# shionhonda/IaGo

Hardware: AMD Instinct MI355X
Metric: self-play games/sec (higher is better)
Workload: dtype f16 MFMA operands (float32 split in 2 / 3 pieces), f32 accumulate; u64 bitboards; f32 / f64 tree statistics

## Files before the change

iago_amd/csrc/conv_policy_body.hpp:

```cpp
#pragma once
#include "abi_common.hpp"
#include "search_request.hpp"

#include <hip/hip_fp16.h>

#include <cstdlib>

#include <atomic>

namespace iago_policy {


typedef _Float16 half8 __attribute__((ext_vector_type(8)));
typedef float float16v __attribute__((ext_vector_type(16)));
typedef float float4v __attribute__((ext_vector_type(4)));
#define IAGO_POLICY_MFMA16(acc, a, b) asm volatile("v_mfma_f32_16x16x32_f16 %0, %1, %2, %0" : "+a"(acc) : "v"(a), "v"(b))
typedef unsigned int u32x4 __attribute__((ext_vector_type(4)));
typedef float f2 __attribute__((ext_vector_type(2)));
typedef _Float16 h2 __attribute__((ext_vector_type(2)));

constexpr int RS = 800;
constexpr int ZB = 1280;
constexpr int BS = 64 * RS + ZB;
constexpr int HEAD_FLOATS = 64;
constexpr int W1_LDS = (64 * 18 + 64) * 4;
constexpr int LDS_BYTES = BS + 1024 + HEAD_FLOATS * 4 + W1_LDS;
constexpr float S1 = 1.0f / 2048.0f, S2 = 1.0f / (2048.0f * 2048.0f);

struct PolicyParams {
    const uint64_t *own, *opp;
    const int64_t *index;
    const int32_t *n_dev;
    int64_t n;
    const float *w1, *b1;
    const uint4 *w_hi[7], *w_mid[7], *w_lo[7];
    const float *bias[7];
    const float *w9, *b10;
    float *probs;
    uint32_t *overflow;
    int layer_lo, layer_hi;
    uint4 *scratch;
    int64_t row_lo, row_hi;
};

__device__ __forceinline__ void split3(const f2 v, h2 &hi, h2 &mid, h2 &lo)
{
    hi = __builtin_convertvector(v, h2);
    const f2 r1 = (v - __builtin_convertvector(hi, f2)) * 2048.0f;
    mid = __builtin_convertvector(r1, h2);
    const f2 r2 = (r1 - __builtin_convertvector(mid, f2)) * 2048.0f;
    lo = __builtin_convertvector(r2, h2);
}

extern __shared__ __align__(16) char policy_lds[];

template <bool SRCH = false>
__device__ __forceinline__ void policy_item(const PolicyParams &P, const int64_t row_id, const uint32_t *pos = nullptr,
                                            float *res = nullptr, const float *w1_staged = nullptr,
                                            const float *head_w = nullptr)
{
    char *const T = policy_lds;
    int tid_ = threadIdx.x;
    if constexpr (SRCH)
        asm volatile("" : "+v"(tid_));
    const int tid = tid_, wv = __builtin_amdgcn_readfirstlane(tid >> 6), lane = tid & 63;
    const int64_t b = P.index ? P.index[row_id] : row_id;

    if (tid < ZB / 16)
        *(uint4 *)(T + 64 * RS + tid * 16) = make_uint4(0, 0, 0, 0);
    bool saturated = false;
    if (P.layer_lo > 0) {
        const uint4 *src = P.scratch + (row_id - P.row_lo) * (64 * RS / 16);
        for (int e = tid; e < 64 * RS / 16; e += 256)
            *(uint4 *)(T + e * 16) = src[e];
    } else {
        const int cell = tid & 63, y = cell >> 3, x = cell & 7;
        const uint64_t bits0 = SRCH ? iago_request::opp(pos) : P.opp[b];
        const uint64_t bits1 = SRCH ? iago_request::own(pos) : P.own[b];
        float in[18];
#pragma unroll
        for (int c = 0; c < 2; c++)
#pragma unroll
            for (int ky = 0; ky < 3; ky++)
#pragma unroll
                for (int kx = 0; kx < 3; kx++) {
                    const int yy = y + ky - 1, xx = x + kx - 1;
                    const bool ok = yy >= 0 && yy < 8 && xx >= 0 && xx < 8;
                    const int a = (yy * 8 + xx) & 63;
                    in[c * 9 + ky * 3 + kx] = (ok && (((c ? bits1 : bits0) >> a) & 1ull)) ? 1.0f : 0.0f;
                }
        const float *w1s = w1_staged;
        if constexpr (!SRCH) {
            float *const st = (float *)(T + BS + 1024 + HEAD_FLOATS * 4);
            for (int e = tid; e < 64 * 18 / 4; e += 256)
                ((float4 *)st)[e] = ((const float4 *)P.w1)[e];
            if (tid < 16)
                ((float4 *)(st + 64 * 18))[tid] = ((const float4 *)P.b1)[tid];
            __syncthreads();
            w1s = st;
        }
#pragma unroll 1
        for (int g2 = 0; g2 < 2; g2++) {
            const int grp = __builtin_amdgcn_readfirstlane(g2 * 4 + wv);
            const int co0 = grp * 8;
            _Float16 p0[8], p1[8], p2[8];
#pragma unroll
            for (int k = 0; k < 8; k += 2) {
                const float *wa = w1s + (co0 + k) * 18, *wb = wa + 18;
                f2 acc = (f2){w1s[64 * 18 + co0 + k], w1s[64 * 18 + co0 + k + 1]};
#pragma unroll
                for (int j = 0; j < 18; j++)
                    acc = __builtin_elementwise_fma((f2){wa[j], wb[j]}, (f2){in[j], in[j]}, acc);
                saturated |= !(acc.x <= 65000.0f) || !(acc.y <= 65000.0f);
                f2 v;
                v.x = fminf(fmaxf(acc.x, 0.0f), 65000.0f);
                v.y = fminf(fmaxf(acc.y, 0.0f), 65000.0f);
                h2 a0, a1, a2;
                split3(v, a0, a1, a2);
                p0[k] = a0.x, p0[k + 1] = a0.y;
                p1[k] = a1.x, p1[k + 1] = a1.y;
                p2[k] = a2.x, p2[k + 1] = a2.y;
            }
            char *dst = T + cell * RS + (grp >> 1) * 32 + (grp & 1) * 16;
            *(uint4 *)dst = *(const uint4 *)p0;
            *(uint4 *)(dst + 256) = *(const uint4 *)p1;
            *(uint4 *)(dst + 512) = *(const uint4 *)p2;
        }
    }
    __syncthreads();

    const int c16 = lane & 15, kq = lane >> 4;
    uint32_t addr[4][9];
#pragma unroll
    for (int q = 0; q < 4; q++)
#pragma unroll
        for (int tap = 0; tap < 9; tap++) {
            const int cell = 16 * q + c16;
            const int yy = (cell >> 3) + tap / 3 - 1, xx = (cell & 7) + tap % 3 - 1;
            const bool ok = yy >= 0 && yy < 8 && xx >= 0 && xx < 8;
            const int lin = (cell + (tap / 3 - 1) * 8 + (tap % 3 - 1)) & 7;
            addr[q][tap] = (uint32_t)((ok ? (yy * 8 + xx) * RS : 64 * RS + 32 * lin) + kq * 16);
        }
    uint32_t wrow[4];
#pragma unroll
    for (int q = 0; q < 4; q++)
        wrow[q] = (uint32_t)((16 * q + c16) * RS);

    for (int L = P.layer_lo; L < P.layer_hi; L++) {
        const int n_pairs = L == 0 ? 2 : 4;
        const char *const wh = (const char *)P.w_hi[L], *const wm = (const char *)P.w_mid[L], *const wl = (const char *)P.w_lo[L];
        const uint32_t a_lane = (uint32_t)(((32 * wv + c16) * 2 + (kq & 1) + (kq >> 1) * (9 * 256)) * 16);
        auto a_load = [&](const char *base, uint32_t step_bytes, int m) -> u32x4 {
            return *(const u32x4 *)(base + step_bytes + a_lane + (uint32_t)m * 512u);
        };
        float4v acc0[2][4], acc0b[2][4], acc1[2][4], acc2[2][4];
#pragma unroll
        for (int m = 0; m < 2; m++)
#pragma unroll
            for (int n = 0; n < 4; n++)
#pragma unroll
                for (int v = 0; v < 4; v++) {
                    acc0[m][n][v] = 0.0f;
                    acc0b[m][n][v] = 0.0f;
                    acc1[m][n][v] = 0.0f;
                    acc2[m][n][v] = 0.0f;
                }
        u32x4 a_hi[3][2], a_mid[3][2], a_lo[3][2];
#pragma unroll
        for (int i = 0; i < 2; i++)
#pragma unroll
            for (int m = 0; m < 2; m++) {
                a_hi[i][m] = a_load(wh, (uint32_t)i * 4096u, m);
                a_mid[i][m] = a_load(wm, (uint32_t)i * 4096u, m);
                a_lo[i][m] = a_load(wl, (uint32_t)i * 4096u, m);
            }
        half8 bh[3], bm[3], bl[3];
        auto b_addr = [&](int tile) -> const char * {
            const int over = tile >= 36 ? 64 : 0, tt = tile % 36;
            return T + addr[tt & 3][tt >> 2] + over;
        };
        {
            const char *p0 = b_addr(0), *p1 = b_addr(1);
            bh[0] = *(const half8 *)p0, bm[0] = *(const half8 *)(p0 + 256), bl[0] = *(const half8 *)(p0 + 512);
            bh[1] = *(const half8 *)p1, bm[1] = *(const half8 *)(p1 + 256), bl[1] = *(const half8 *)(p1 + 512);
        }
        for (int cp = 0; cp < n_pairs; cp++) {
#pragma unroll
            for (int tap = 0; tap < 9; tap++) {
                int cp2 = cp, tp2 = tap + 2;
                if (tp2 >= 9) {
                    tp2 -= 9;
                    cp2 += 1;
                }
                if (cp2 >= n_pairs) {
                    cp2 = n_pairs - 1;
                    tp2 = 8;
                }
                const uint32_t w2 = (uint32_t)(18 * cp2 + tp2) * 4096u;
                half8 ah[2], am[2], al[2];
#pragma unroll
                for (int m = 0; m < 2; m++) {
                    ah[m] = __builtin_bit_cast(half8, a_hi[tap % 3][m]);
                    am[m] = __builtin_bit_cast(half8, a_mid[tap % 3][m]);
                    al[m] = __builtin_bit_cast(half8, a_lo[tap % 3][m]);
                }
#pragma unroll
                for (int q = 0; q < 4; q++) {
                    const int tile = tap * 4 + q, cur = tile % 3, nxt = (tile + 2) % 3;
                    const char *p = b_addr(tile + 2);
                    __builtin_amdgcn_sched_barrier(0);
                    IAGO_POLICY_MFMA16(acc2[0][q], ah[0], bl[cur]);
                    bh[nxt] = *(const half8 *)p;
                    __builtin_amdgcn_sched_barrier(0);
                    IAGO_POLICY_MFMA16(acc2[1][q], ah[1], bl[cur]);
                    bm[nxt] = *(const half8 *)(p + 256);
                    __builtin_amdgcn_sched_barrier(0);
                    IAGO_POLICY_MFMA16(acc1[0][q], ah[0], bm[cur]);
                    bl[nxt] = *(const half8 *)(p + 512);
                    __builtin_amdgcn_sched_barrier(0);
                    IAGO_POLICY_MFMA16(acc1[1][q], ah[1], bm[cur]);
                    if (q == 0)
                        a_hi[(tap + 2) % 3][0] = a_load(wh, w2, 0);
                    else if (q == 1)
                        a_mid[(tap + 2) % 3][0] = a_load(wm, w2, 0);
                    else if (q == 2)
                        a_lo[(tap + 2) % 3][0] = a_load(wl, w2, 0);
                    __builtin_amdgcn_sched_barrier(0);
                    if (tap & 1)
                        IAGO_POLICY_MFMA16(acc0b[0][q], ah[0], bh[cur]);
                    else
                        IAGO_POLICY_MFMA16(acc0[0][q], ah[0], bh[cur]);
                    if (q == 0)
                        a_hi[(tap + 2) % 3][1] = a_load(wh, w2, 1);
                    else if (q == 1)
                        a_mid[(tap + 2) % 3][1] = a_load(wm, w2, 1);
                    else if (q == 2)
                        a_lo[(tap + 2) % 3][1] = a_load(wl, w2, 1);
                    __builtin_amdgcn_sched_barrier(0);
                    if (tap & 1)
                        IAGO_POLICY_MFMA16(acc0b[1][q], ah[1], bh[cur]);
                    else
                        IAGO_POLICY_MFMA16(acc0[1][q], ah[1], bh[cur]);
                    IAGO_POLICY_MFMA16(acc2[0][q], al[0], bh[cur]);
                    IAGO_POLICY_MFMA16(acc2[1][q], al[1], bh[cur]);
                    IAGO_POLICY_MFMA16(acc1[0][q], am[0], bh[cur]);
                    IAGO_POLICY_MFMA16(acc1[1][q], am[1], bh[cur]);
                    IAGO_POLICY_MFMA16(acc2[0][q], am[0], bm[cur]);
                    IAGO_POLICY_MFMA16(acc2[1][q], am[1], bm[cur]);
                    __builtin_amdgcn_sched_barrier(0);
                }
            }
#pragma unroll
            for (int q = 0; q < 4; q++)
#pragma unroll
                for (int tap = 0; tap < 9; tap++)
                    addr[q][tap] += 64u;
        }
#pragma unroll
        for (int q = 0; q < 4; q++)
#pragma unroll
            for (int tap = 0; tap < 9; tap++)
                addr[q][tap] -= 64u * (uint32_t)n_pairs;

        f2 bia[2][2];
#pragma unroll
        for (int m = 0; m < 2; m++) {
            const float4 bq = *(const float4 *)(P.bias[L] + 32 * wv + 16 * m + 4 * kq);
            bia[m][0] = (f2){bq.x, bq.y};
            bia[m][1] = (f2){bq.z, bq.w};
        }
        asm volatile("s_nop 15\n\ts_nop 7" ::: "memory");
        __syncthreads();
        float vmax = 0.0f;
        f2 vsum = (f2){0.0f, 0.0f};
#pragma unroll
        for (int q = 0; q < 4; q++) {
            char *row = T + wrow[q] + (32 * wv + 4 * kq) * 2;
#pragma unroll
            for (int m = 0; m < 2; m++) {
                h2 p0[2], p1[2], p2[2];
#pragma unroll
                for (int t2 = 0; t2 < 2; t2++) {
                    const f2 m0 = (f2){acc0[m][q][2 * t2], acc0[m][q][2 * t2 + 1]} + (f2){acc0b[m][q][2 * t2], acc0b[m][q][2 * t2 + 1]};
                    const f2 m1 = (f2){acc1[m][q][2 * t2], acc1[m][q][2 * t2 + 1]};
                    const f2 m2 = (f2){acc2[m][q][2 * t2], acc2[m][q][2 * t2 + 1]};
                    f2 v = (m2 * S2 + m1 * S1) + m0 + bia[m][t2];
                    vmax = fmaxf(fmaxf(vmax, v.x), v.y);
                    vsum += v;
                    v.x = __builtin_amdgcn_fmed3f(v.x, 0.0f, 65000.0f);
                    v.y = __builtin_amdgcn_fmed3f(v.y, 0.0f, 65000.0f);
                    split3(v, p0[t2], p1[t2], p2[t2]);
                }
                *(uint2 *)(row + 32 * m) = (uint2){__builtin_bit_cast(uint32_t, p0[0]), __builtin_bit_cast(uint32_t, p0[1])};
                *(uint2 *)(row + 32 * m + 256) =
                    (uint2){__builtin_bit_cast(uint32_t, p1[0]), __builtin_bit_cast(uint32_t, p1[1])};
                *(uint2 *)(row + 32 * m + 512) =
                    (uint2){__builtin_bit_cast(uint32_t, p2[0]), __builtin_bit_cast(uint32_t, p2[1])};
            }
        }
        saturated |= !(vmax <= 65000.0f) || !(vsum.x + vsum.y == vsum.x + vsum.y);
        __syncthreads();
    }
    if (P.overflow && saturated)
        *P.overflow = 1u;
    if (P.layer_hi < 7) {
        uint4 *dst = P.scratch + (row_id - P.row_lo) * (64 * RS / 16);
        for (int e = tid; e < 64 * RS / 16; e += 256)
            dst[e] = *(const uint4 *)(T + e * 16);
        return;
    }

    if (wv == 0) {
        const char *row = T + lane * RS;
        float acc = 0.0f;
#pragma unroll 4
        for (int c8 = 0; c8 < 16; c8++) {
            const half8 xh = *(const half8 *)(row + c8 * 16), xm = *(const half8 *)(row + 256 + c8 * 16),
                        xl = *(const half8 *)(row + 512 + c8 * 16);
            const float *w9 = SRCH ? head_w : P.w9;
            const float4 wa = *(const float4 *)(w9 + c8 * 8), wb = *(const float4 *)(w9 + c8 * 8 + 4);
            const float w[8] = {wa.x, wa.y, wa.z, wa.w, wb.x, wb.y, wb.z, wb.w};
#pragma unroll
            for (int e = 0; e < 8; e++) {
                const float xv = ((float)xl[e] * S2 + (float)xm[e] * S1) + (float)xh[e];
                acc = fmaf(w[e], xv, acc);
            }
        }
        const float logit = acc + (SRCH ? head_w[128 + lane] : P.b10[lane]);
        float mx = logit;
#pragma unroll
        for (int o = 32; o > 0; o >>= 1)
            mx = fmaxf(mx, __shfl_xor(mx, o));
        const float e = expf(logit - mx);
        float sum = e;
#pragma unroll
        for (int o = 32; o > 0; o >>= 1)
            sum += __shfl_xor(sum, o);
        if constexpr (SRCH)
            res[lane] = e / sum;
        else
            P.probs[row_id * 64 + lane] = e / sum;
    }
}

inline int policy_params_of(const iago_policy_split3_args *a, PolicyParams &P)
{
    if (!a || a->n < 0)
        return iago_fail(IAGO_ERR_INVALID, "iago_policy_forward_split3: null args or n < 0");
    if (!a->own || !a->opp || !a->w1 || !a->b1 || !a->w9 || !a->b10 || !a->probs)
        return iago_fail(IAGO_ERR_INVALID, "iago_policy_forward_split3: null pointer");
    for (int L = 0; L < 7; L++) {
        if (!a->w_hi[L] || !a->w_mid[L] || !a->w_lo[L] || !a->bias[L] || ((uintptr_t)a->w_hi[L] & 15u) ||
            ((uintptr_t)a->w_mid[L] & 15u) || ((uintptr_t)a->w_lo[L] & 15u) || ((uintptr_t)a->bias[L] & 15u))
            return iago_fail(IAGO_ERR_INVALID, "iago_policy_forward_split3: weights and biases of blocks 2..8 must be "
                                               "non-null and 16-byte aligned");
        P.w_hi[L] = (const uint4 *)a->w_hi[L];
        P.w_mid[L] = (const uint4 *)a->w_mid[L];
        P.w_lo[L] = (const uint4 *)a->w_lo[L];
        P.bias[L] = a->bias[L];
    }
    if (((uintptr_t)a->w9 & 15u) || ((uintptr_t)a->w1 & 15u) || ((uintptr_t)a->b1 & 15u))
        return iago_fail(IAGO_ERR_INVALID, "iago_policy_forward_split3: w1, b1, w9 must be 16-byte aligned");
    P.own = a->own;
    P.opp = a->opp;
    P.index = a->index;
    P.n_dev = a->n_dev;
    P.n = a->n;
    P.w1 = a->w1;
    P.b1 = a->b1;
    P.w9 = a->w9;
    P.b10 = a->b10;
    P.probs = a->probs;
    P.overflow = a->overflow;
    P.layer_lo = 0;
    P.layer_hi = 7;
    P.scratch = nullptr;
    P.row_lo = 0;
    P.row_hi = a->n;
    return IAGO_OK;
}

}
```

iago_amd/csrc/conv_trunk_body.hpp:

```cpp
#pragma once
#include "abi_common.hpp"
#include "rollout_row_body.hpp"
#include "search_request.hpp"

#include <hip/hip_fp16.h>

#include <atomic>
#include <type_traits>

namespace iago_trunk {


typedef _Float16 half8 __attribute__((ext_vector_type(8)));
typedef float float16v __attribute__((ext_vector_type(16)));
typedef float float4v __attribute__((ext_vector_type(4)));
typedef unsigned int u32x4 __attribute__((ext_vector_type(4)));
typedef float f2 __attribute__((ext_vector_type(2)));
typedef _Float16 h2 __attribute__((ext_vector_type(2)));

constexpr int RS = 544;
constexpr int ZB = 1024;
constexpr int BS = 64 * RS + ZB;
constexpr int lds_alloc(int tb) { return tb * BS + 1024; }
constexpr int MAX_LAYERS = 8;

#define IAGO_MFMA16(acc, a, b) asm volatile("v_mfma_f32_16x16x32_f16 %0, %1, %2, %0" : "+a"(acc) : "v"(a), "v"(b))

struct TrunkRParams {
    const uint4 *x_hi, *x_lo;
    uint4 *y_hi, *y_lo;
    const uint4 *w_hi[MAX_LAYERS], *w_lo[MAX_LAYERS];
    const float *bias[MAX_LAYERS];
    int64_t n;
    int32_t cin0, n_layers;
    uint32_t *overflow;
    const float *planes;
    const uint64_t *own, *opp;
    const float *w1, *b1;
    const uint4 *w9_hi, *w9_lo;
    const float *b9, *w10, *w11;
    float *out;
    const int64_t *index;
    const int32_t *n_dev;
    int32_t count_lo, count_hi;
    int32_t layer_lo, layer_hi;
    char *scratch;
};
constexpr int IMG = 64 * RS;

struct Piece {
    const int64_t *index;
    const int32_t *n_dev;
    char *scratch;
    int layer_lo, layer_hi;
    const uint32_t *pos;
    float *res;
    const float *w1s;
    const char *head_w;
};
constexpr int HEAD_W_W9LO = 8192, HEAD_W_W10 = 16384, HEAD_W_W11 = 16384 + 32768, HEAD_W_B9 = HEAD_W_W11 + 512,
              HEAD_W_LDS = HEAD_W_B9 + 16;
__device__ __forceinline__ Piece whole_walk(const TrunkRParams &P)
{
    return Piece{P.index, P.n_dev, P.scratch, P.layer_lo, P.layer_hi, nullptr, nullptr, nullptr, nullptr};
}

constexpr int head_lds(int tb) { return (9 * 64 * tb + 64 * tb + 128 * tb) * 4; }
constexpr int W1_LDS = (64 * 18 + 64) * 4;
constexpr int lds_alloc_fused(int tb) { return lds_alloc(tb) + head_lds(tb) + W1_LDS; }

__device__ __forceinline__ int cell_of_lane(int r)
{
    return r < 4 ? r : r < 12 ? 16 + (r - 4) : r < 16 ? 4 + (r - 12) : r < 20 ? 24 + (r - 16) : r < 28 ? 8 + (r - 20)
                                                                                              : 28 + (r - 28);
}

extern __shared__ __align__(16) char trunk_lds[];

constexpr bool tile_off_board(int tb, int tap, int n)
{
    return tb >= 2 && ((tap < 3 && (n & 7) == 0) || (tap >= 6 && (n & 7) == 7));
}
constexpr int kept_before(int tb, int tap, int n)
{
    int k = 0;
    for (int t = 0; t < 9; t++)
        for (int m = 0; m < 4 * tb; m++) {
            if (t == tap && m == n)
                return k;
            k += !tile_off_board(tb, t, m);
        }
    return k;
}
constexpr int kept_tile(int tb, int k)
{
    for (int t = 0; t < 9; t++)
        for (int m = 0; m < 4 * tb; m++)
            if (!tile_off_board(tb, t, m) && k-- == 0)
                return t * 4 * tb + m;
    return -1;
}
template <int I0, int I1, class F>
__device__ __forceinline__ void static_for(F &&f)
{
    if constexpr (I0 < I1) {
        f(std::integral_constant<int, I0>{});
        static_for<I0 + 1, I1>(f);
    }
}

template <bool FUSED, int TB, bool SRCH = false>
__device__ __forceinline__ void trunk_item(const TrunkRParams &P, const Piece &W, const int64_t b0, const int64_t n_rows)
{
    constexpr int NN = 4 * TB;
    char *const T = trunk_lds;
    int tid_ = threadIdx.x;
    if constexpr (SRCH)
        asm volatile("" : "+v"(tid_));
    const int tid = tid_, wv = __builtin_amdgcn_readfirstlane(tid >> 6), lane = tid & 63, r = lane & 31, h = lane >> 5;

    if (tid < TB * (ZB / 16))
        *(uint4 *)(T + (tid / (ZB / 16)) * BS + 64 * RS + (tid % (ZB / 16)) * 16) = make_uint4(0, 0, 0, 0);
    bool saturated = false;
    constexpr bool PIECES = FUSED && TB <= 2;
    if (PIECES && W.layer_lo > 0) {
        constexpr int PER = (TB * (IMG / 16) + 255) / 256;
        uint4 img[PER];
#pragma unroll
        for (int i = 0; i < PER; i++) {
            const int e = min(tid + i * 256, TB * (IMG / 16) - 1);
            const int board = e / (IMG / 16), off = e - board * (IMG / 16);
            const int64_t row = min(b0 + board, n_rows - 1);
            img[i] = ((const uint4 *)(W.scratch + row * IMG))[off];
        }
#pragma unroll
        for (int i = 0; i < PER; i++) {
            const int e = tid + i * 256;
            const int board = e / (IMG / 16), off = e - board * (IMG / 16);
            if (e < TB * (IMG / 16))
                *(uint4 *)(T + board * BS + off * 16) = img[i];
        }
    } else if constexpr (FUSED) {
        const int cell = tid & 63, y = cell >> 3, x = cell & 7;
        float in[TB][18];
#pragma unroll
        for (int board = 0; board < TB; board++) {
            const int64_t row = min(b0 + board, n_rows - 1);
            const int64_t b = W.index ? W.index[row] : row;
            const float *pl = P.planes + b * 128;
            uint64_t bits0, bits1;
            if constexpr (SRCH) {
                const uint32_t *w = W.pos + iago_request::WORDS * board;
                bits1 = iago_request::own(w);
                bits0 = iago_request::opp(w);
            } else {
                bits0 = P.planes ? 0ull : P.opp[b];
                bits1 = P.planes ? 0ull : P.own[b];
            }
#pragma unroll
            for (int c = 0; c < 2; c++)
#pragma unroll
                for (int ky = 0; ky < 3; ky++)
#pragma unroll
                    for (int kx = 0; kx < 3; kx++) {
                        const int yy = y + ky - 1, xx = x + kx - 1;
                        const bool ok = yy >= 0 && yy < 8 && xx >= 0 && xx < 8;
                        const int a = (yy * 8 + xx) & 63;
                        float v;
                        if (P.planes)
                            v = ok ? pl[c * 64 + a] : 0.0f;
                        else
                            v = (ok && (((c ? bits1 : bits0) >> a) & 1ull)) ? 1.0f : 0.0f;
                        in[board][c * 9 + ky * 3 + kx] = v;
                    }
        }
        const float *w1s = W.w1s;
        if constexpr (!SRCH) {
            float *const st = (float *)(T + lds_alloc(TB) + head_lds(TB));
            for (int e = tid; e < 64 * 18 / 4; e += 256)
                ((float4 *)st)[e] = ((const float4 *)P.w1)[e];
            if (tid < 16)
                ((float4 *)(st + 64 * 18))[tid] = ((const float4 *)P.b1)[tid];
            __syncthreads();
            w1s = st;
        }
#pragma unroll 1
        for (int g2 = 0; g2 < 2; g2++) {
            const int grp = __builtin_amdgcn_readfirstlane(g2 * 4 + wv);
            const int co0 = grp * 8;
            _Float16 h8[TB][8], l8[TB][8];
#pragma unroll
            for (int k = 0; k < 8; k++) {
                const float *wk = w1s + (co0 + k) * 18;
                const float bk = w1s[64 * 18 + co0 + k];
                float wreg[18];
#pragma unroll
                for (int j = 0; j < 18; j++)
                    wreg[j] = wk[j];
                float accs[TB];
                if constexpr (TB % 2 == 0) {
#pragma unroll
                    for (int bp = 0; bp < TB; bp += 2) {
                        f2 acc = (f2){bk, bk};
#pragma unroll
                        for (int j = 0; j < 18; j++)
                            acc = __builtin_elementwise_fma((f2){wreg[j], wreg[j]}, (f2){in[bp][j], in[bp + 1][j]}, acc);
                        accs[bp] = acc.x;
                        accs[bp + 1] = acc.y;
                    }
                } else {
#pragma unroll
                    for (int board = 0; board < TB; board++) {
                        float acc = bk;
#pragma unroll
                        for (int j = 0; j < 18; j++)
                            acc = fmaf(wreg[j], in[board][j], acc);
                        accs[board] = acc;
                    }
                }
#pragma unroll
                for (int board = 0; board < TB; board++) {
                    const float acc = accs[board];
                    saturated |= !(acc <= 65000.0f);
                    const float v = fminf(fmaxf(acc, 0.0f), 65000.0f);
                    const _Float16 vh = (_Float16)v;
                    h8[board][k] = vh;
                    l8[board][k] = (_Float16)((v - (float)vh) * 2048.0f);
                }
            }
#pragma unroll
            for (int board = 0; board < TB; board++) {
                char *dst = T + board * BS + cell * RS + (grp >> 1) * 32 + (grp & 1) * 16;
                *(uint4 *)dst = *(const uint4 *)h8[board];
                *(uint4 *)(dst + 256) = *(const uint4 *)l8[board];
            }
        }
    } else {
        const int chunks0 = P.cin0 >> 4;
        const int pieces = TB * chunks0 * 128;
        for (int e = tid; e < pieces; e += 256) {
            const int board = e / (chunks0 * 128), rem = e - board * chunks0 * 128;
            const int chunk = rem >> 7, cell = (rem >> 1) & 63, hp = rem & 1;
            const int64_t b = min(b0 + board, P.n - 1);
            const int64_t src = (b * chunks0 + chunk) * 128 + (rem & 127);
            char *dst = T + board * BS + cell * RS + chunk * 32 + hp * 16;
            *(uint4 *)dst = P.x_hi[src];
            *(uint4 *)(dst + 256) = P.x_lo[src];
        }
    }
    __syncthreads();

    constexpr bool ROWS = TB >= 2;
    static_assert(TB == 1 || TB == 2 || TB == 4, "boards per workgroup");
    const int c16 = lane & 15, kq = lane >> 4;
    constexpr int NADDR = ROWS ? 9 : 36;
    uint32_t addr[NADDR];
    uint32_t sx[2] = {0u, 0u};
    uint32_t wrow[ROWS ? 1 : 4];
    if constexpr (ROWS) {
        const int x = c16 & 7, odd = c16 >> 3;
#pragma unroll
        for (int tap = 0; tap < 9; tap++) {
            const int row = tap < 3 ? 1 : 0;
            const int yy = row + tap / 3 - 1, xx = x + tap % 3 - 1;
            const bool ok = xx >= 0 && xx < 8;
            addr[tap] = (uint32_t)(odd * BS + (ok ? (yy * 8 + xx) * RS : 64 * RS + 32 * (xx & 7)) + kq * 16);
        }
        sx[0] = x > 0 ? 8u * RS : 0u;
        sx[1] = x < 7 ? 8u * RS : 0u;
        wrow[0] = (uint32_t)(odd * BS + x * RS);
    } else {
#pragma unroll
        for (int q = 0; q < 4; q++)
#pragma unroll
            for (int tap = 0; tap < 9; tap++) {
                const int cell = 16 * q + c16;
                const int yy = (cell >> 3) + tap / 3 - 1, xx = (cell & 7) + tap % 3 - 1;
                const bool ok = yy >= 0 && yy < 8 && xx >= 0 && xx < 8;
                const int lin = (cell + (tap / 3 - 1) * 8 + (tap % 3 - 1)) & 7;
                addr[9 * q + tap] = (uint32_t)((ok ? (yy * 8 + xx) * RS : 64 * RS + 32 * lin) + kq * 16);
            }
#pragma unroll
        for (int q = 0; q < 4; q++)
            wrow[q] = (uint32_t)((16 * q + c16) * RS);
    }
    auto b_off = [&](int tap, int n) -> uint32_t {
        if constexpr (ROWS) {
            const int dx = tap % 3 - 1, r = (n & 7) - (tap < 3 ? 1 : 0);
            return addr[tap] + (uint32_t)r * (dx == 0 ? 8u * RS : sx[dx > 0]) + (uint32_t)(n >> 3) * (2u * BS);
        } else {
            return addr[9 * n + tap];
        }
    };

    const int L_lo = PIECES ? W.layer_lo : 0, L_hi = PIECES ? W.layer_hi : P.n_layers;
    for (int L = L_lo; L < L_hi; L++) {
        const int n_pairs = L == 0 ? (P.cin0 >> 5) : 4;
        const char *const wh = (const char *)P.w_hi[L], *const wl = (const char *)P.w_lo[L];
        const uint32_t a_lane = (uint32_t)(((32 * wv + c16) * 2 + (kq & 1) + (kq >> 1) * (9 * 256)) * 16);
        auto a_load = [&](const char *base, uint32_t step_bytes, int m) -> u32x4 {
            return *(const u32x4 *)(base + step_bytes + a_lane + (uint32_t)m * 512u);
        };
        float4v acc_main[2][NN], acc_cross[2][NN];
#pragma unroll
        for (int m = 0; m < 2; m++)
#pragma unroll
            for (int n = 0; n < NN; n++)
#pragma unroll
                for (int v = 0; v < 4; v++) {
                    acc_main[m][n][v] = 0.0f;
                    acc_cross[m][n][v] = 0.0f;
                }

        u32x4 a_hi[3][2], a_lo[3][2];
#pragma unroll
        for (int i = 0; i < 2; i++)
#pragma unroll
            for (int m = 0; m < 2; m++) {
                a_hi[i][m] = a_load(wh, (uint32_t)i * 4096u, m);
                a_lo[i][m] = a_load(wl, (uint32_t)i * 4096u, m);
            }
        constexpr int KEPT = kept_before(TB, 9, 0), NR = KEPT % 4 == 0 ? 4 : 6;
        static_assert(KEPT % NR == 0, "the B ring must line up at every chunk pair");
        half8 bh[NR], bl[NR];
        static_for<0, 3>([&](auto kc) __attribute__((always_inline)) {
            constexpr int tile = kept_tile(TB, decltype(kc)::value);
            const char *p0 = T + b_off(tile / NN, tile % NN);
            bh[decltype(kc)::value] = *(const half8 *)p0;
            bl[decltype(kc)::value] = *(const half8 *)(p0 + 256);
        });
        for (int cp = 0; cp < n_pairs; cp++) {
            static_for<0, KEPT>([&](auto kc) __attribute__((always_inline)) {
                constexpr int k = decltype(kc)::value, tile = kept_tile(TB, k), tap = tile / NN, n = tile % NN;
                constexpr int j = k - kept_before(TB, tap, 0);
                static_assert(kept_before(TB, tap + 1, 0) - kept_before(TB, tap, 0) >= 4, "four A loads per k-step");
                constexpr int kn = k + 3, tile_n = kept_tile(TB, kn % KEPT), cur = k % NR, nxt = kn % NR;
                constexpr uint32_t over = kn >= KEPT ? 64u : 0u;
                int cp2 = cp, tp2 = tap + 2;
                if (tp2 >= 9) {
                    tp2 -= 9;
                    cp2 += 1;
                }
                if (cp2 >= n_pairs) {
                    cp2 = n_pairs - 1;
                    tp2 = 8;
                }
                const uint32_t w2 = (uint32_t)(18 * cp2 + tp2) * 4096u;
                const half8 ah0 = __builtin_bit_cast(half8, a_hi[tap % 3][0]), ah1 = __builtin_bit_cast(half8, a_hi[tap % 3][1]);
                const half8 al0 = __builtin_bit_cast(half8, a_lo[tap % 3][0]), al1 = __builtin_bit_cast(half8, a_lo[tap % 3][1]);
                const char *p = T + b_off(tile_n / NN, tile_n % NN) + over;
                __builtin_amdgcn_sched_barrier(0);
                IAGO_MFMA16(acc_cross[0][n], ah0, bl[cur]);
                bh[nxt] = *(const half8 *)p;
                __builtin_amdgcn_sched_barrier(0);
                IAGO_MFMA16(acc_cross[1][n], ah1, bl[cur]);
                bl[nxt] = *(const half8 *)(p + 256);
                __builtin_amdgcn_sched_barrier(0);
                IAGO_MFMA16(acc_main[0][n], ah0, bh[cur]);
                if constexpr (j == 0)
                    a_hi[(tap + 2) % 3][0] = a_load(wh, w2, 0);
                else if constexpr (j == 1)
                    a_hi[(tap + 2) % 3][1] = a_load(wh, w2, 1);
                else if constexpr (j == 2)
                    a_lo[(tap + 2) % 3][0] = a_load(wl, w2, 0);
                else if constexpr (j == 3)
                    a_lo[(tap + 2) % 3][1] = a_load(wl, w2, 1);
                __builtin_amdgcn_sched_barrier(0);
                IAGO_MFMA16(acc_main[1][n], ah1, bh[cur]);
                IAGO_MFMA16(acc_cross[0][n], al0, bh[cur]);
                IAGO_MFMA16(acc_cross[1][n], al1, bh[cur]);
                __builtin_amdgcn_sched_barrier(0);
            });
#pragma unroll
            for (int i = 0; i < NADDR; i++)
                addr[i] += 64u;
        }
#pragma unroll
        for (int i = 0; i < NADDR; i++)
            addr[i] -= 64u * (uint32_t)n_pairs;

        f2 bia[2][2];
#pragma unroll
        for (int m = 0; m < 2; m++) {
            const float4 bq = *(const float4 *)(P.bias[L] + 32 * wv + 16 * m + 4 * kq);
            bia[m][0] = (f2){bq.x, bq.y};
            bia[m][1] = (f2){bq.z, bq.w};
        }
        asm volatile("s_nop 15\n\ts_nop 7" ::: "memory");
        __syncthreads();
        float vmax = 0.0f;
        f2 vsum = (f2){0.0f, 0.0f};
#pragma unroll
        for (int n = 0; n < NN; n++) {
            char *row = T + (ROWS ? wrow[0] + (n & 7) * (8 * RS) + (n >> 3) * (2 * BS) : wrow[ROWS ? 0 : n]) + (32 * wv + 4 * kq) * 2;
#pragma unroll
            for (int m = 0; m < 2; m++) {
                h2 hi[2], lo[2];
#pragma unroll
                for (int t2 = 0; t2 < 2; t2++) {
                    const f2 mm = (f2){acc_main[m][n][2 * t2], acc_main[m][n][2 * t2 + 1]};
                    const f2 c = (f2){acc_cross[m][n][2 * t2], acc_cross[m][n][2 * t2 + 1]};
                    f2 v = c * (1.0f / 2048.0f) + mm + bia[m][t2];
                    vmax = fmaxf(fmaxf(vmax, v.x), v.y);
                    vsum += v;
                    v.x = __builtin_amdgcn_fmed3f(v.x, 0.0f, 65000.0f);
                    v.y = __builtin_amdgcn_fmed3f(v.y, 0.0f, 65000.0f);
                    hi[t2] = __builtin_convertvector(v, h2);
                    lo[t2] = __builtin_convertvector((v - __builtin_convertvector(hi[t2], f2)) * 2048.0f, h2);
                }
                *(uint2 *)(row + 32 * m) = (uint2){__builtin_bit_cast(uint32_t, hi[0]), __builtin_bit_cast(uint32_t, hi[1])};
                *(uint2 *)(row + 32 * m + 256) =
                    (uint2){__builtin_bit_cast(uint32_t, lo[0]), __builtin_bit_cast(uint32_t, lo[1])};
            }
        }
        saturated |= !(vmax <= 65000.0f) || !(vsum.x + vsum.y == vsum.x + vsum.y);
        __syncthreads();
    }
    if (P.overflow && saturated)
        *P.overflow = 1u;

    if (PIECES && W.layer_hi < P.n_layers) {
        for (int e = tid; e < TB * (IMG / 16); e += 256) {
            const int board = e / (IMG / 16), off = e - board * (IMG / 16);
            if (b0 + board < n_rows)
                ((uint4 *)(W.scratch + (b0 + board) * IMG))[off] = *(const uint4 *)(T + board * BS + off * 16);
        }
        return;
    }
    if constexpr (FUSED) {
        constexpr int NC = 64 * TB;
        float *const Dm = (float *)(T + lds_alloc(TB));
        float *const h9s = Dm + 9 * NC;
        float *const hid = h9s + NC;
        float4 w10row[16];
        if constexpr (!SRCH) {
#pragma unroll
            for (int c = 0; c < 16; c++)
                w10row[c] = ((const float4 *)(P.w10 + (tid & 127) * 64))[c];
        }
        const float w11j = SRCH ? ((const float *)(W.head_w + HEAD_W_W11))[tid & 127] : P.w11[tid & 127];
        const float b9 = SRCH ? *(const float *)(W.head_w + HEAD_W_B9) : P.b9[0];
        const int lane_cell = cell_of_lane(r);
        if (wv < TB) {
            const u32x4 *w9h = (const u32x4 *)P.w9_hi + r * 2 + h;
            const u32x4 *w9l = (const u32x4 *)P.w9_lo + r * 2 + h;
            float16v hm[2], hc[2];
#pragma unroll
            for (int jt = 0; jt < 2; jt++)
#pragma unroll
                for (int v = 0; v < 16; v++) {
                    hm[jt][v] = 0.0f;
                    hc[jt][v] = 0.0f;
                }
            u32x4 w9a[SRCH ? 1 : 8], w9b[SRCH ? 1 : 8];
            if constexpr (!SRCH) {
#pragma unroll
                for (int c = 0; c < 8; c++) {
                    w9a[c] = w9h[c * 64];
                    w9b[c] = w9l[c * 64];
                }
            }
#pragma unroll
            for (int c = 0; c < 8; c++) {
                const half8 ah = SRCH ? *(const half8 *)(W.head_w + (c * 64 + r * 2 + h) * 16)
                                      : __builtin_bit_cast(half8, w9a[SRCH ? 0 : c]);
                const half8 al = SRCH ? *(const half8 *)(W.head_w + HEAD_W_W9LO + (c * 64 + r * 2 + h) * 16)
                                      : __builtin_bit_cast(half8, w9b[SRCH ? 0 : c]);
#pragma unroll
                for (int jt = 0; jt < 2; jt++) {
                    const int jj = 2 * wv + jt;
                    const char *p = T + (jj >> 1) * BS + (32 * (jj & 1) + lane_cell) * RS + h * 16 + c * 32;
                    const half8 bh9 = *(const half8 *)p, bl9 = *(const half8 *)(p + 256);
                    hm[jt] = __builtin_amdgcn_mfma_f32_32x32x16_f16(ah, bh9, hm[jt], 0, 0, 0);
                    hc[jt] = __builtin_amdgcn_mfma_f32_32x32x16_f16(ah, bl9, hc[jt], 0, 0, 0);
                    hc[jt] = __builtin_amdgcn_mfma_f32_32x32x16_f16(al, bh9, hc[jt], 0, 0, 0);
                }
            }
#pragma unroll
            for (int jt = 0; jt < 2; jt++) {
                const int jj = 2 * wv + jt;
                const int base = (jj >> 1) * 64 + 32 * (jj & 1) + lane_cell;
#pragma unroll
                for (int t = 0; t < 4; t++)
                    Dm[(4 * h + t) * NC + base] = hm[jt][t] + hc[jt][t] * (1.0f / 2048.0f);
                if (h == 0)
                    Dm[8 * NC + base] = hm[jt][4] + hc[jt][4] * (1.0f / 2048.0f);
            }
        }
        __syncthreads();
        if constexpr (SRCH) {
#pragma unroll
            for (int c = 0; c < 16; c++)
                w10row[c] = ((const float4 *)(W.head_w + HEAD_W_W10))[c * 128 + (tid & 127)];
        }
        if (tid < NC) {
            const int cell = tid & 63, y = cell >> 3, x = cell & 7;
            float s9 = 0.0f;
#pragma unroll
            for (int tap = 0; tap < 9; tap++) {
                const int yy = y + tap / 3 - 1, xx = x + tap % 3 - 1;
                if (yy >= 0 && yy < 8 && xx >= 0 && xx < 8)
                    s9 += Dm[tap * NC + (tid & ~63) + yy * 8 + xx];
            }
            h9s[tid] = fmaxf(s9 + b9, 0.0f);
        }
        __syncthreads();
        if ((tid >> 7) * 2 < TB) {
            const int j = tid & 127, pb = (tid >> 7) * 2;
            float s0 = 0.0f, s1 = 0.0f;
#pragma unroll
            for (int c = 0; c < 16; c++) {
                const float4 wq = w10row[c];
                const float4 x0 = *(const float4 *)(h9s + pb * 64 + 4 * c);
                const float4 x1 = *(const float4 *)(h9s + (pb + 1 < TB ? pb + 1 : pb) * 64 + 4 * c);
                s0 = fmaf(wq.x, x0.x, s0);
                s0 = fmaf(wq.y, x0.y, s0);
                s0 = fmaf(wq.z, x0.z, s0);
                s0 = fmaf(wq.w, x0.w, s0);
                s1 = fmaf(wq.x, x1.x, s1);
                s1 = fmaf(wq.y, x1.y, s1);
                s1 = fmaf(wq.z, x1.z, s1);
                s1 = fmaf(wq.w, x1.w, s1);
            }
            hid[pb * 128 + j] = s0 * w11j;
            if (pb + 1 < TB)
                hid[(pb + 1) * 128 + j] = s1 * w11j;
        }
        __syncthreads();
        if (tid < TB && b0 + tid < n_rows) {
            float4 hv[32];
#pragma unroll
            for (int j4 = 0; j4 < 32; j4++)
                hv[j4] = *(const float4 *)(hid + tid * 128 + 4 * j4);
            float v = 0.0f;
#pragma unroll
            for (int j4 = 0; j4 < 32; j4++) {
#pragma clang fp reassociate(off)
                v += hv[j4].x;
                v += hv[j4].y;
                v += hv[j4].z;
                v += hv[j4].w;
            }
            const int64_t row = b0 + tid;
            if constexpr (SRCH)
                W.res[tid] = v;
            else
                P.out[W.index ? W.index[row] : row] = v;
        }
        return;
    }
    for (int e = tid; e < TB * 1024; e += 256) {
        const int board = e >> 10, cb = (e >> 7) & 7, cell = (e >> 1) & 63, hp = e & 1;
        const int64_t b = b0 + board;
        if (b < P.n) {
            const char *src = T + board * BS + cell * RS + cb * 32 + hp * 16;
            P.y_hi[b * 1024 + (e & 1023)] = *(const uint4 *)src;
            P.y_lo[b * 1024 + (e & 1023)] = *(const uint4 *)(src + 256);
        }
    }
}

template <bool FUSED, int TB>
__device__ __forceinline__ void trunk_walk(const TrunkRParams &P, const Piece &W, const int64_t bid, const int64_t nb)
{
    int64_t n_rows = P.n;
    if constexpr (FUSED) {
        if (W.n_dev)
            n_rows = min(P.n, (int64_t)*W.n_dev);
        if (n_rows <= P.count_lo || n_rows > P.count_hi)
            return;
    }
    for (int64_t b0 = bid * TB; b0 < n_rows; b0 += nb * TB) {
        trunk_item<FUSED, TB>(P, W, b0, n_rows);
        __syncthreads();
    }
}

inline int value_params_of(const iago_value_split_args *a, TrunkRParams &P)
{
    if (!a || a->n < 0)
        return iago_fail(IAGO_ERR_INVALID, "iago_value_forward_split: null args or n < 0");
    if ((!a->planes && (!a->own || !a->opp)) || !a->w1 || !a->b1 || !a->w9_hi || !a->w9_lo || !a->b9 || !a->w10 ||
        !a->w11 || !a->out)
        return iago_fail(IAGO_ERR_INVALID, "iago_value_forward_split: null pointer");
    for (int L = 0; L < 7; L++) {
        if (!a->w_hi[L] || !a->w_lo[L] || !a->bias[L] || ((uintptr_t)a->w_hi[L] & 15u) || ((uintptr_t)a->w_lo[L] & 15u) ||
            ((uintptr_t)a->bias[L] & 15u))
            return iago_fail(IAGO_ERR_INVALID, "iago_value_forward_split: weights and biases of blocks 2..8 must be "
                                               "non-null and 16-byte aligned");
        P.w_hi[L] = (const uint4 *)a->w_hi[L];
        P.w_lo[L] = (const uint4 *)a->w_lo[L];
        P.bias[L] = a->bias[L];
    }
    P.w_hi[7] = P.w_hi[6];
    P.w_lo[7] = P.w_lo[6];
    P.bias[7] = P.bias[6];
    if (((uintptr_t)a->w9_hi & 15u) || ((uintptr_t)a->w9_lo & 15u) || ((uintptr_t)a->w10 & 15u) || ((uintptr_t)a->w1 & 15u) ||
        ((uintptr_t)a->b1 & 15u))
        return iago_fail(IAGO_ERR_INVALID, "iago_value_forward_split: w1, b1, w9_hi, w9_lo, w10 must be 16-byte aligned");
    P.x_hi = P.x_lo = nullptr;
    P.y_hi = P.y_lo = nullptr;
    P.n = a->n;
    P.cin0 = 64;
    P.n_layers = 7;
    P.overflow = a->overflow;
    P.planes = a->planes;
    P.own = a->own;
    P.opp = a->opp;
    P.w1 = a->w1;
    P.b1 = a->b1;
    P.w9_hi = (const uint4 *)a->w9_hi;
    P.w9_lo = (const uint4 *)a->w9_lo;
    P.b9 = a->b9;
    P.w10 = a->w10;
    P.w11 = a->w11;
    P.out = a->out;
    if (a->index && a->planes)
        return iago_fail(IAGO_ERR_INVALID, "iago_value_forward_split: a gather list needs the boards, not planes");
    P.index = a->index;
    P.n_dev = a->n_dev;
    P.layer_lo = 0;
    P.layer_hi = 7;
    P.scratch = nullptr;
    return IAGO_OK;
}

}
```

Before: 3034.

## Spread policy head reconstruction and value-head MFMA work across all waves

The split3 residual now uses v_fma_mix_f32 to subtract the half piece and rescale in one instruction per lane. In the policy head, all four waves reconstruct the float32 activations from the three half pieces into a float32 LDS buffer before wave 0 does the dot product, instead of wave 0 doing all the reconstruction alone. In the trunk value head with TB==2, each of the four waves handles one 32-cell tile instead of two waves handling two tiles each. The price is two extra barriers and an LDS round trip in the policy head, plus inline asm that depends on op_sel encoding being correct.

```diff
diff --git a/iago_amd/csrc/conv_policy_body.hpp b/iago_amd/csrc/conv_policy_body.hpp
--- a/iago_amd/csrc/conv_policy_body.hpp
+++ b/iago_amd/csrc/conv_policy_body.hpp
@@ -43,12 +43,21 @@
     int64_t row_lo, row_hi;
 };
 
+__device__ __forceinline__ f2 residual(const f2 v, const h2 h)
+{
+    const f2 s = v * 2048.0f;
+    f2 d;
+    asm("v_fma_mix_f32 %0, -%1, %2, %3 op_sel_hi:[1,0,0]" : "=v"(d.x) : "v"(h), "s"(2048.0f), "v"(s.x));
+    asm("v_fma_mix_f32 %0, -%1, %2, %3 op_sel:[1,0,0] op_sel_hi:[1,0,0]" : "=v"(d.y) : "v"(h), "s"(2048.0f), "v"(s.y));
+    return d;
+}
+
 __device__ __forceinline__ void split3(const f2 v, h2 &hi, h2 &mid, h2 &lo)
 {
     hi = __builtin_convertvector(v, h2);
-    const f2 r1 = (v - __builtin_convertvector(hi, f2)) * 2048.0f;
+    const f2 r1 = residual(v, hi);
     mid = __builtin_convertvector(r1, h2);
-    const f2 r2 = (r1 - __builtin_convertvector(mid, f2)) * 2048.0f;
+    const f2 r2 = residual(r1, mid);
     lo = __builtin_convertvector(r2, h2);
 }
 
@@ -310,21 +319,45 @@
         return;
     }
 
+    constexpr int XS = 128 * 4 + 16;
+    static_assert(64 * XS <= 64 * RS, "the float32 rows lie over the image");
+    {
+        const char *row = T + lane * RS;
+        float4 xv4[4][2];
+#pragma unroll
+        for (int i = 0; i < 4; i++) {
+            const int c8 = wv + 4 * i;
+            const half8 xh = *(const half8 *)(row + c8 * 16), xm = *(const half8 *)(row + 256 + c8 * 16),
+                        xl = *(const half8 *)(row + 512 + c8 * 16);
+            float xv[8];
+#pragma unroll
+            for (int e = 0; e < 8; e++)
+                xv[e] = ((float)xl[e] * S2 + (float)xm[e] * S1) + (float)xh[e];
+            xv4[i][0] = make_float4(xv[0], xv[1], xv[2], xv[3]);
+            xv4[i][1] = make_float4(xv[4], xv[5], xv[6], xv[7]);
+        }
+        __syncthreads();
+#pragma unroll
+        for (int i = 0; i < 4; i++) {
+            float4 *dst = (float4 *)(T + lane * XS + (wv + 4 * i) * 32);
+            dst[0] = xv4[i][0];
+            dst[1] = xv4[i][1];
+        }
+        __syncthreads();
+    }
     if (wv == 0) {
-        const char *row = T + lane * RS;
+        const char *row = T + lane * XS;
         float acc = 0.0f;
 #pragma unroll 4
         for (int c8 = 0; c8 < 16; c8++) {
-            const half8 xh = *(const half8 *)(row + c8 * 16), xm = *(const half8 *)(row + 256 + c8 * 16),
-                        xl = *(const half8 *)(row + 512 + c8 * 16);
+            const float4 xa = *(const float4 *)(row + c8 * 32), xb = *(const float4 *)(row + c8 * 32 + 16);
+            const float xv[8] = {xa.x, xa.y, xa.z, xa.w, xb.x, xb.y, xb.z, xb.w};
             const float *w9 = SRCH ? head_w : P.w9;
             const float4 wa = *(const float4 *)(w9 + c8 * 8), wb = *(const float4 *)(w9 + c8 * 8 + 4);
             const float w[8] = {wa.x, wa.y, wa.z, wa.w, wb.x, wb.y, wb.z, wb.w};
 #pragma unroll
-            for (int e = 0; e < 8; e++) {
-                const float xv = ((float)xl[e] * S2 + (float)xm[e] * S1) + (float)xh[e];
-                acc = fmaf(w[e], xv, acc);
-            }
+            for (int e = 0; e < 8; e++)
+                acc = fmaf(w[e], xv[e], acc);
         }
         const float logit = acc + (SRCH ? head_w[128 + lane] : P.b10[lane]);
         float mx = logit;
diff --git a/iago_amd/csrc/conv_trunk_body.hpp b/iago_amd/csrc/conv_trunk_body.hpp
--- a/iago_amd/csrc/conv_trunk_body.hpp
+++ b/iago_amd/csrc/conv_trunk_body.hpp
@@ -441,12 +441,13 @@
         const float w11j = SRCH ? ((const float *)(W.head_w + HEAD_W_W11))[tid & 127] : P.w11[tid & 127];
         const float b9 = SRCH ? *(const float *)(W.head_w + HEAD_W_B9) : P.b9[0];
         const int lane_cell = cell_of_lane(r);
-        if (wv < TB) {
+        constexpr int JT = TB == 2 ? 1 : 2;
+        if (TB == 2 || wv < TB) {
             const u32x4 *w9h = (const u32x4 *)P.w9_hi + r * 2 + h;
             const u32x4 *w9l = (const u32x4 *)P.w9_lo + r * 2 + h;
-            float16v hm[2], hc[2];
-#pragma unroll
-            for (int jt = 0; jt < 2; jt++)
+            float16v hm[JT], hc[JT];
+#pragma unroll
+            for (int jt = 0; jt < JT; jt++)
 #pragma unroll
                 for (int v = 0; v < 16; v++) {
                     hm[jt][v] = 0.0f;
@@ -467,8 +468,8 @@
                 const half8 al = SRCH ? *(const half8 *)(W.head_w + HEAD_W_W9LO + (c * 64 + r * 2 + h) * 16)
                                       : __builtin_bit_cast(half8, w9b[SRCH ? 0 : c]);
 #pragma unroll
-                for (int jt = 0; jt < 2; jt++) {
-                    const int jj = 2 * wv + jt;
+                for (int jt = 0; jt < JT; jt++) {
+                    const int jj = JT * wv + jt;
                     const char *p = T + (jj >> 1) * BS + (32 * (jj & 1) + lane_cell) * RS + h * 16 + c * 32;
                     const half8 bh9 = *(const half8 *)p, bl9 = *(const half8 *)(p + 256);
                     hm[jt] = __builtin_amdgcn_mfma_f32_32x32x16_f16(ah, bh9, hm[jt], 0, 0, 0);
@@ -477,8 +478,8 @@
                 }
             }
 #pragma unroll
-            for (int jt = 0; jt < 2; jt++) {
-                const int jj = 2 * wv + jt;
+            for (int jt = 0; jt < JT; jt++) {
+                const int jj = JT * wv + jt;
                 const int base = (jj >> 1) * 64 + 32 * (jj & 1) + lane_cell;
 #pragma unroll
                 for (int t = 0; t < 4; t++)
```

New measurement: 3032 (median of 2 runs). No clear change (-0.1%).
